# Manta-Network/manta-rs

Hardware: AMD Instinct MI355X
Metric: G1 MSM Mscalar/s at 2^20 (higher is better)
Workload: dtype u32; 1 GPU; 2^20 BLS12-381 G1 variable-base MSM per GPU, uniform scalars resident in HBM; curve=BLS12-381, log_n=20, window_bits=17, msms_in_flight=3

## Files before the change

manta_rs_amd/csrc/ec_dev.h:

```cpp
#pragma once
#include "fp_dev.h"

namespace mg {

#define MG_EC_CALL __device__ __noinline__

template <class F, int B> struct Bv {
    F v;
};
template <int B, class F> MG_DEV Bv<F, B> bv(const F &f) { return Bv<F, B>{f}; }
template <class F, int A, int B> MG_DEV Bv<F, F::BM> operator*(const Bv<F, A> &a, const Bv<F, B> &b) {
    static_assert((long)A * B * F::MULK <= F::LIM, "product of operand bounds exceeds the Montgomery headroom");
    return Bv<F, F::BM>{F::template mulb<A, B>(a.v, b.v)};
}
template <class F, int A> MG_DEV Bv<F, F::BM> b_sqr(const Bv<F, A> &a) {
    static_assert((long)A * A * F::MULK <= F::LIM, "square of operand bound exceeds the Montgomery headroom");
    return Bv<F, F::BM>{F::template sqrb<A>(a.v)};
}
template <class F, int A, int B> MG_DEV Bv<F, A + B> operator+(const Bv<F, A> &a, const Bv<F, B> &b) {
    return Bv<F, A + B>{F::add(a.v, b.v)};
}
template <class F, int A> MG_DEV Bv<F, 2 * A> b_dbl(const Bv<F, A> &a) { return Bv<F, 2 * A>{F::dbl(a.v)}; }
template <class F, int A, int B> MG_DEV Bv<F, A + B> operator-(const Bv<F, A> &a, const Bv<F, B> &b) {
    static_assert(B <= F::MAXM, "no multiple of p large enough for this subtrahend");
    return Bv<F, A + B>{F::template sub<B>(a.v, b.v)};
}
template <class F, int A, int B, int C>
MG_DEV Bv<F, A + B + 2 * C> b_sub2(const Bv<F, A> &a, const Bv<F, B> &b, const Bv<F, C> &c) {
    static_assert(B + 2 * C <= F::MAXM, "no multiple of p large enough for this subtrahend");
    return Bv<F, A + B + 2 * C>{F::template sub2<B + 2 * C>(a.v, b.v, c.v)};
}
template <class F, int A> MG_DEV Bv<F, A> b_neg(const Bv<F, A> &a) {
    static_assert(A <= F::MAXM, "no multiple of p large enough");
    return Bv<F, A>{F::template neg<A>(a.v)};
}
template <class F, int A> MG_DEV bool b_is_zero(const Bv<F, A> &a) {
    static_assert(A - 1 <= F::MAXM, "multiple table too short for this zero test");
    return a.v.template is_zero_mod<A>();
}
template <int T, class F, int A> MG_DEV Bv<F, T> b_fit(const Bv<F, A> &a) {
    if constexpr (A <= T) {
        return Bv<F, T>{a.v};
    } else {
        static_assert(F::BRED <= T, "reduction cannot reach the requested bound");
        return Bv<F, T>{F::template reduce<A>(a.v)};
    }
}

template <class F> struct Affine {
    F x, y;
    MG_DEV bool is_inf() const { return x.is_zero_exact() && y.is_zero_exact(); }
    static MG_DEV Affine load(const u32 *p) { return Affine{F::load_aff(p), F::load_aff(p + F::AFF_N)}; }
    MG_DEV void store(u32 *p) const {
        x.store_aff(p);
        y.store_aff(p + F::AFF_N);
    }
    static constexpr int WORDS = 2 * F::AFF_N;
};

template <class F> struct XYZZ {
    F x, y, zz, zzz;
    static constexpr int WORDS = 4 * F::N;
    static constexpr int BX = F::BX, BY = F::BY, BM = F::BM;
    MG_DEV bool is_inf() const { return zz.is_zero_exact(); }
    static MG_DEV XYZZ inf() { return XYZZ{F::zero(), F::zero(), F::zero(), F::zero()}; }
    static MG_DEV XYZZ from_affine(const Affine<F> &a) {
        if (a.is_inf()) return inf();
        return XYZZ{a.x, a.y, F::one(), F::one()};
    }
    static MG_DEV XYZZ load(const u32 *p) {
        return XYZZ{F::load(p), F::load(p + F::N), F::load(p + 2 * F::N), F::load(p + 3 * F::N)};
    }
    MG_DEV void store(u32 *p) const {
        x.store(p);
        y.store(p + F::N);
        zz.store(p + 2 * F::N);
        zzz.store(p + 3 * F::N);
    }
    MG_DEV void store_std(u32 *p) const {
        typedef typename F::Std S;
        x.to_std().store(p);
        y.to_std().store(p + S::N);
        zz.to_std().store(p + 2 * S::N);
        zzz.to_std().store(p + 3 * S::N);
    }
    static MG_DEV XYZZ shfl(const XYZZ &a, int src) {
        return XYZZ{F::shfl(a.x, src), F::shfl(a.y, src), F::shfl(a.zz, src), F::shfl(a.zzz, src)};
    }
    static MG_DEV XYZZ select(bool c, const XYZZ &a, const XYZZ &b) {
        return XYZZ{F::select(c, a.x, b.x), F::select(c, a.y, b.y), F::select(c, a.zz, b.zz), F::select(c, a.zzz, b.zzz)};
    }

    template <int AX, int AY>
    static MG_DEV void dbl_core(const Bv<F, AX> &px, const Bv<F, AY> &py, F &X3o, F &Y3o, F &Vo, F &Wo) {
        auto U = b_fit<8>(b_dbl(py));
        auto V = b_sqr(U);
        auto W = U * V;
        auto S = px * V;
        auto X2 = b_sqr(px);
        auto M = b_fit<6>(b_dbl(X2) + X2);
        auto X3 = b_fit<BX>(b_sub2(b_sqr(M), bv<0>(F::zero()), S));
        auto Y3 = b_fit<BY>(M * (S - X3) - W * py);
        X3o = X3.v;
        Y3o = Y3.v;
        Vo = V.v;
        Wo = W.v;
    }
    static MG_EC_CALL XYZZ dbl_affine_call(const Affine<F> &p) { return dbl_affine_body(p); }
    static MG_DEV XYZZ dbl_affine(const Affine<F> &p) {
        if constexpr (F::EXT) return dbl_affine_call(p);
        else return dbl_affine_body(p);
    }
    static MG_DEV XYZZ dbl_affine_body(const Affine<F> &p) {
        XYZZ r;
        dbl_core(bv<BM>(p.x), bv<BM>(p.y), r.x, r.y, r.zz, r.zzz);
        return r;
    }
    static MG_EC_CALL XYZZ dbl_call(const XYZZ &p) { return dbl_body(p); }
    static MG_DEV XYZZ dbl(const XYZZ &p) {
        if constexpr (F::EXT) return dbl_call(p);
        else return dbl_body(p);
    }
    static MG_DEV XYZZ dbl_body(const XYZZ &p) {
        if (p.is_inf()) return p;
        XYZZ r;
        F V, W;
        dbl_core(bv<BX>(p.x), bv<BY>(p.y), r.x, r.y, V, W);
        r.zz = (bv<BM>(V) * bv<BM>(p.zz)).v;
        r.zzz = (bv<BM>(W) * bv<BM>(p.zzz)).v;
        return r;
    }
    MG_EC_CALL void madd_call(const Affine<F> &q, bool neg) { madd_body(q, neg); }
    MG_DEV void madd(const Affine<F> &q, bool neg) {
        if constexpr (F::EXT) madd_call(q, neg);
        else madd_body(q, neg);
    }
    MG_DEV void madd_throughput(const Affine<F> &q, bool neg) {
        if constexpr (!F::EXT && F::LAZY) {
#ifdef MG_ACC_TWO_CHAINS
            madd_lazy<false>(q, neg);
#else
            madd_lazy<true>(q, neg);
#endif
            return;
        }
        madd(q, neg);
    }
    template <bool CH = false> MG_DEV void madd_lazy(const Affine<F> &q_in, bool negate) {
        static_assert(!F::EXT && F::LAZY, "reduced-radix base field only");
        static_assert(F::BX == 8 && F::BY == 4 && F::BM == 2 && F::LIM >= 121, "bound analysis above");
        constexpr bool LL = F::LAZY_LIMBS;
        if (q_in.is_inf()) return;
        F qy = q_in.y;
        if (negate) {
            if constexpr (LL) qy = F::template negl<3>(q_in.y);
            else qy = F::template neg<2>(q_in.y);
        }
        if (is_inf()) {
            x = q_in.x;
            y = negate ? F::template neg<2>(q_in.y) : q_in.y;
            zz = F::one();
            zzz = F::one();
            return;
        }
        const F U2 = F::template mul_t<CH>(q_in.x, zz);
        const F S2 = F::template mul_t<CH>(qy, zzz);
        F P, R;
        if constexpr (LL) {
            P = F::template subl<9>(U2, x);
            R = F::template subl<5>(S2, y);
        } else {
            P = F::template sub<8>(U2, x);
            R = F::template sub<4>(S2, y);
        }
        const F PP = F::template sqr_t<CH>(P);
        if (PP.template is_zero_mod<2>()) {
            if ((LL ? F::normalize_u(R) : R).template is_zero_mod<7>()) {
                Affine<F> q{q_in.x, negate ? F::template neg<2>(q_in.y) : q_in.y};
                *this = dbl_affine(q);
            } else {
                *this = inf();
            }
            return;
        }
        const F PPP = F::template mul_t<CH>(P, PP);
        const F Q = F::template mul_t<CH>(x, PP);
        const F X3 = F::template sub2<6>(F::template sqr_t<CH>(R), PPP, Q);
        F T, N;
        if constexpr (LL) {
            T = F::template subl<9>(Q, X3);
            N = F::template negl<3>(PPP);
        } else {
            T = F::template sub<8>(Q, X3);
            N = F::template neg<2>(PPP);
        }
        const F Y3 = F::template mul_add_t<CH>(R, T, y, N);
        zz = F::template mul_t<CH>(zz, PP);
        zzz = F::template mul_t<CH>(zzz, PPP);
        x = X3;
        y = Y3;
    }
    MG_DEV void madd_body(const Affine<F> &q_in, bool negate) {
        if constexpr (!F::EXT && F::LAZY) {
            madd_lazy<false>(q_in, negate);
            return;
        }
        if (q_in.is_inf()) return;
        Affine<F> q = q_in;
        if (negate) q.y = b_neg(bv<BM>(q.y)).v;
        if (is_inf()) {
            x = q.x;
            y = q.y;
            zz = F::one();
            zzz = F::one();
            return;
        }
        const auto X1 = bv<BX>(x);
        const auto Y1 = bv<BY>(y);
        const auto ZZ1 = bv<BM>(zz);
        const auto ZZZ1 = bv<BM>(zzz);
        auto U2 = bv<BM>(q.x) * ZZ1;
        auto S2 = bv<BM>(q.y) * ZZZ1;
        auto P = U2 - X1;
        auto R = S2 - Y1;
        if (b_is_zero(P)) {
            if (b_is_zero(R))
                *this = dbl_affine(q);
            else
                *this = inf();
            return;
        }
        auto PP = b_sqr(P);
        auto PPP = P * PP;
        auto Q = X1 * PP;
        auto X3 = b_fit<BX>(b_sub2(b_sqr(R), PPP, Q));
        auto Y3 = b_fit<BY>(R * (Q - X3) - Y1 * PPP);
        x = X3.v;
        y = Y3.v;
        zz = (ZZ1 * PP).v;
        zzz = (ZZZ1 * PPP).v;
    }
    MG_EC_CALL void add_call(const XYZZ &o) { add_body(o); }
    MG_DEV void add(const XYZZ &o) {
        if constexpr (F::EXT) add_call(o);
        else add_body(o);
    }
    MG_DEV void add_body(const XYZZ &o) {
        if (o.is_inf()) return;
        if (is_inf()) {
            *this = o;
            return;
        }
        auto U1 = bv<BX>(x) * bv<BM>(o.zz);
        auto U2 = bv<BX>(o.x) * bv<BM>(zz);
        auto S1 = bv<BY>(y) * bv<BM>(o.zzz);
        auto S2 = bv<BY>(o.y) * bv<BM>(zzz);
        auto P = U2 - U1;
        auto R = S2 - S1;
        if (b_is_zero(P)) {
            if (b_is_zero(R))
                *this = dbl(*this);
            else
                *this = inf();
            return;
        }
        auto PP = b_sqr(P);
        auto PPP = P * PP;
        auto Q = U1 * PP;
        auto X3 = b_fit<BX>(b_sub2(b_sqr(R), PPP, Q));
        auto Y3 = b_fit<BY>(R * (Q - X3) - S1 * PPP);
        x = X3.v;
        y = Y3.v;
        zz = ((bv<BM>(zz) * bv<BM>(o.zz)) * PP).v;
        zzz = ((bv<BM>(zzz) * bv<BM>(o.zzz)) * PPP).v;
    }
};

template <class F, bool ALLOW_DOUBLE = true> struct CoopAdd {
    static constexpr int SLOT = F::XWORDS;
    static constexpr bool DOUBLE = ALLOW_DOUBLE && 2 * 4 * SLOT * 4 <= 49152;
    static constexpr int LDS_WORDS = (DOUBLE ? 2 : 1) * 4 * SLOT;
    static MG_DEV void swap(u32 *buf, int wave, int lane, const F &mine, F (&all)[4]) {
        mine.store_x(buf + wave * SLOT, lane);
        __syncthreads();
#pragma unroll
        for (int q = 0; q < 4; ++q) all[q] = F::load_x(buf + q * SLOT, lane);
        if (!DOUBLE) __syncthreads();
    }
    static MG_DEV void add(XYZZ<F> &acc, const XYZZ<F> &o, u32 *lds, int wave, int lane) {
        constexpr int BX = F::BX, BY = F::BY, BM = F::BM;
        const bool o_inf = o.is_inf(), a_inf = acc.is_inf();
        F mine, r[4];
        if (wave == 0) mine = (bv<BX>(acc.x) * bv<BM>(o.zz)).v;
        else if (wave == 1) mine = (bv<BX>(o.x) * bv<BM>(acc.zz)).v;
        else if (wave == 2) mine = (bv<BY>(acc.y) * bv<BM>(o.zzz)).v;
        else mine = (bv<BY>(o.y) * bv<BM>(acc.zzz)).v;
        swap(lds, wave, lane, mine, r);
        const auto U1 = bv<BM>(r[0]), U2 = bv<BM>(r[1]), S1 = bv<BM>(r[2]), S2 = bv<BM>(r[3]);
        const auto P = U2 - U1;
        const auto R = S2 - S1;
        const bool p0 = b_is_zero(P), r0 = b_is_zero(R);
        if (wave == 0) mine = b_sqr(P).v;
        else if (wave == 1) mine = b_sqr(R).v;
        else if (wave == 2) mine = (bv<BM>(acc.zz) * bv<BM>(o.zz)).v;
        else mine = (bv<BM>(acc.zzz) * bv<BM>(o.zzz)).v;
        swap(lds + (DOUBLE ? 4 * SLOT : 0), wave, lane, mine, r);
        const auto PP = bv<BM>(r[0]), RR = bv<BM>(r[1]), Z12 = bv<BM>(r[2]), Z123 = bv<BM>(r[3]);
        if (wave == 0) mine = (P * PP).v;
        else if (wave == 1) mine = (U1 * PP).v;
        else if (wave == 2) mine = (Z12 * PP).v;
        else mine = F::zero();
        swap(lds, wave, lane, mine, r);
        const auto PPP = bv<BM>(r[0]), Q = bv<BM>(r[1]);
        const F ZZ3 = r[2];
        const auto X3 = b_fit<BX>(b_sub2(RR, PPP, Q));
        if (wave == 0) mine = (R * (Q - X3)).v;
        else if (wave == 1) mine = (S1 * PPP).v;
        else if (wave == 2) mine = (Z123 * PPP).v;
        else mine = F::zero();
        swap(lds + (DOUBLE ? 4 * SLOT : 0), wave, lane, mine, r);
        const auto Y3 = b_fit<BY>(bv<BM>(r[0]) - bv<BM>(r[1]));
        XYZZ<F> sum{X3.v, Y3.v, ZZ3, r[2]};
        if (o_inf) {
            sum = acc;
        } else if (a_inf) {
            sum = o;
        } else if (p0) {
            if (r0) sum = XYZZ<F>::dbl(acc);
            else sum = XYZZ<F>::inf();
        }
        acc = sum;
    }
};

}
```

manta_rs_amd/csrc/msm_reduce.h:

```cpp
#pragma once
#include "msm_common.h"

namespace mg {

template <class F>
__global__ __launch_bounds__(256) MG_TAIL_ATTR void merge_partials(u32 *__restrict__ pkeys, u32 *__restrict__ ppts, u32 cnt, u32 G,
                                                      u32 invalid, int final_level, u32 *__restrict__ buckets,
                                                      u32 *__restrict__ okeys, u32 *__restrict__ opts, u32 n_waves,
                                                      u32 *__restrict__ std_final) {
    MG_PRIO_FOR(F);
    constexpr size_t XW = XYZZ<F>::WORDS;
    const u32 wave = blockIdx.x * (blockDim.x >> 6) + (threadIdx.x >> 6);
    const int lane = threadIdx.x & 63;
    if (wave >= n_waves) return;
    const size_t b = ((size_t)wave * 64 + lane) * G;
    u32 kh = invalid, kt = invalid;
    bool single = true;
    XYZZ<F> acc = XYZZ<F>::inf();
    if (b < cnt) {
        const size_t end = b + G < cnt ? b + G : cnt;
        u32 cur = pkeys[b];
        if (cur != invalid) {
            kh = cur;
            acc = XYZZ<F>::load(ppts + b * XW);
            for (size_t j = b + 1; j < end; ++j) {
                const u32 k = pkeys[j];
                if (k != cur) {
                    if (single) {
                        acc.store(ppts + b * XW);
                        single = false;
                    } else {
                        acc.store(buckets + (size_t)cur * XW);
                    }
                    cur = k;
                    acc = XYZZ<F>::inf();
                    if (k == invalid) break;
                    acc = XYZZ<F>::load(ppts + j * XW);
                } else {
                    const XYZZ<F> p = XYZZ<F>::load(ppts + j * XW);
                    if (!p.is_inf()) acc.add(p);
                }
            }
            kt = cur;
        }
    }
    for (int d = 1; d < 64; d <<= 1) {
        const u32 nk = __shfl_up(kt, d, 64);
        const bool take = (lane >= d) && (nk == kt) && (kt != invalid);
        if (!__any(take)) break;
        const XYZZ<F> o = XYZZ<F>::shfl(acc, lane - d < 0 ? lane : lane - d);
        if (take) acc.add(o);
    }
    const u32 prev_kt = __shfl_up(kt, 1, 64), next_kh = __shfl_down(kh, 1, 64);
    const u32 key0 = __shfl(kh, 0, 64);
    const bool need_in = !single && lane > 0 && prev_kt == kh;
    const bool any_in = __any(need_in);
    XYZZ<F> prev = XYZZ<F>::inf();
    if (any_in) prev = XYZZ<F>::shfl(acc, lane > 0 ? lane - 1 : 0);
    const bool cont = lane < 63 && next_kh == kt;
    if (kt != invalid && !cont) {
        if (final_level) {
            if (std_final) acc.store_std(std_final + (size_t)kt * XYZZ<typename F::Std>::WORDS);
            else acc.store(buckets + (size_t)kt * XW);
        } else if (kt == key0) {
            okeys[2 * wave] = kt;
            acc.store(opts + (size_t)(2 * wave) * XW);
            if (lane == 63) {
                okeys[2 * wave + 1] = kt;
                XYZZ<F>::inf().store(opts + (size_t)(2 * wave + 1) * XW);
            }
        } else if (lane == 63) {
            okeys[2 * wave + 1] = kt;
            acc.store(opts + (size_t)(2 * wave + 1) * XW);
        } else {
            acc.store(buckets + (size_t)kt * XW);
        }
    }
    if (!final_level && lane == 63 && kt == invalid) {
        okeys[2 * wave + 1] = invalid;
        if (key0 == invalid) okeys[2 * wave] = invalid;
    }
    if (!single) {
        XYZZ<F> h = XYZZ<F>::load(ppts + b * XW);
        if (need_in) h.add(prev);
        if (!final_level && kh == key0) {
            okeys[2 * wave] = kh;
            h.store(opts + (size_t)(2 * wave) * XW);
        } else if (final_level && std_final) {
            h.store_std(std_final + (size_t)kh * XYZZ<typename F::Std>::WORDS);
        } else {
            h.store(buckets + (size_t)kh * XW);
        }
    }
}

template <class F>
__global__ __launch_bounds__(256) MG_TAIL_COOP_ATTR void merge_partials_coop(u32 *__restrict__ pkeys, u32 *__restrict__ ppts, u32 cnt, u32 G,
                                                           u32 invalid, int final_level, u32 *__restrict__ buckets,
                                                           u32 *__restrict__ okeys, u32 *__restrict__ opts,
                                                           u32 *__restrict__ std_final) {
    MG_PRIO_FOR(F);
    __shared__ __attribute__((aligned(16))) u32 lds[CoopAdd<F>::LDS_WORDS];
    constexpr size_t XW = XYZZ<F>::WORDS;
    const u32 wave = blockIdx.x;
    const int lane = threadIdx.x & 63, pw = threadIdx.x >> 6;
    const bool writer = pw == 0;
    const size_t b = ((size_t)wave * 64 + lane) * G;
    u32 kh = invalid, cur = invalid;
    bool single = true, live = false;
    XYZZ<F> acc = XYZZ<F>::inf();
    if (b < cnt) {
        cur = pkeys[b];
        if (cur != invalid) {
            kh = cur;
            acc = XYZZ<F>::load(ppts + b * XW);
            live = true;
        }
    }
    for (u32 off = 1; off < G; ++off) {
        const size_t j = b + off;
        const bool have = live && j < cnt;
        const u32 k = have ? pkeys[j] : invalid;
        XYZZ<F> p = XYZZ<F>::inf();
        if (have && k != invalid) p = XYZZ<F>::load(ppts + j * XW);
        const bool same = have && k == cur;
        if (have && k != cur) {
            if (writer) acc.store(single ? ppts + b * XW : buckets + (size_t)cur * XW);
            single = false;
            cur = k;
            acc = p;
            if (k == invalid) live = false;
        }
        if (__any(same && !p.is_inf())) {
            const XYZZ<F> o = same ? p : XYZZ<F>::inf();
            CoopAdd<F>::add(acc, o, lds, pw, lane);
        }
    }
    const u32 kt = cur;
    __threadfence_block();
    __syncthreads();
    for (int d = 1; d < 64; d <<= 1) {
        const u32 nk = __shfl_up(kt, d, 64);
        const bool take = (lane >= d) && (nk == kt) && (kt != invalid);
        if (!__any(take)) break;
        XYZZ<F> o = XYZZ<F>::shfl(acc, lane - d < 0 ? lane : lane - d);
        if (!take) o = XYZZ<F>::inf();
        CoopAdd<F>::add(acc, o, lds, pw, lane);
    }
    const u32 prev_kt = __shfl_up(kt, 1, 64), next_kh = __shfl_down(kh, 1, 64);
    const u32 key0 = __shfl(kh, 0, 64);
    const bool need_in = !single && lane > 0 && prev_kt == kh;
    const bool any_in = __any(need_in);
    XYZZ<F> prev = XYZZ<F>::inf();
    if (any_in) prev = XYZZ<F>::shfl(acc, lane > 0 ? lane - 1 : 0);
    const bool cont = lane < 63 && next_kh == kt;
    if (writer && kt != invalid && !cont) {
        if (final_level) {
            if (std_final) acc.store_std(std_final + (size_t)kt * XYZZ<typename F::Std>::WORDS);
            else acc.store(buckets + (size_t)kt * XW);
        } else if (kt == key0) {
            okeys[2 * wave] = kt;
            acc.store(opts + (size_t)(2 * wave) * XW);
            if (lane == 63) {
                okeys[2 * wave + 1] = kt;
                XYZZ<F>::inf().store(opts + (size_t)(2 * wave + 1) * XW);
            }
        } else if (lane == 63) {
            okeys[2 * wave + 1] = kt;
            acc.store(opts + (size_t)(2 * wave + 1) * XW);
        } else {
            acc.store(buckets + (size_t)kt * XW);
        }
    }
    if (writer && !final_level && lane == 63 && kt == invalid) {
        okeys[2 * wave + 1] = invalid;
        if (key0 == invalid) okeys[2 * wave] = invalid;
    }
    XYZZ<F> h = XYZZ<F>::inf();
    if (!single) h = XYZZ<F>::load(ppts + b * XW);
    if (any_in) {
        if (!need_in) prev = XYZZ<F>::inf();
        CoopAdd<F>::add(h, prev, lds, pw, lane);
    }
    if (writer && !single) {
        if (!final_level && kh == key0) {
            okeys[2 * wave] = kh;
            h.store(opts + (size_t)(2 * wave) * XW);
        } else if (final_level && std_final) {
            h.store_std(std_final + (size_t)kh * XYZZ<typename F::Std>::WORDS);
        } else {
            h.store(buckets + (size_t)kh * XW);
        }
    }
}

template <class F>
__global__ __launch_bounds__(256) MG_TAIL_ATTR void tile_reduce(const u32 *__restrict__ in, u32 seg_stride ,
                                                   u32 item_off, u32 n_items, u32 tiles_per_seg, u32 n_waves,
                                                   u32 *__restrict__ outA, u32 *__restrict__ outS, int std_out) {
    MG_PRIO_FOR(F);
    const u32 wave = blockIdx.x * (blockDim.x >> 6) + (threadIdx.x >> 6);
    const int lane = threadIdx.x & 63;
    if (wave >= n_waves) return;
    const u32 seg = wave / tiles_per_seg, tile = wave % tiles_per_seg;
    const u32 idx = tile * 64 + lane;
    XYZZ<F> acc = XYZZ<F>::inf();
    if (idx < n_items) acc = XYZZ<F>::load(in + ((size_t)seg * seg_stride + item_off + idx) * XYZZ<F>::WORDS);
    int top = 1;
    {
        const u32 left = n_items - tile * 64;
        const int lim = left < 64 ? (int)left : 64;
        while (top < lim) top <<= 1;
    }
    for (int d = 1; d < top; d <<= 1) {
        const XYZZ<F> o = XYZZ<F>::shfl(acc, lane + d > 63 ? lane : lane + d);
        if (lane + d < 64) acc.add(o);
    }
    constexpr int SW = XYZZ<typename F::Std>::WORDS;
    if (lane == 0) {
        if (std_out)
            acc.store_std(outA + (size_t)wave * SW);
        else
            acc.store(outA + (size_t)wave * XYZZ<F>::WORDS);
    }
    if (outS) {
        for (int d = top >> 1; d >= 1; d >>= 1) {
            const XYZZ<F> o = XYZZ<F>::shfl(acc, lane + d > 63 ? lane : lane + d);
            if (lane < d) acc.add(o);
        }
        if (lane == 0) {
            if (std_out)
                acc.store_std(outS + (size_t)wave * SW);
            else
                acc.store(outS + (size_t)wave * XYZZ<F>::WORDS);
        }
    }
}

template <class F>
__global__ __launch_bounds__(256) MG_SERIAL_ATTR void serial_reduce(const u32 *__restrict__ in, u32 seg_stride , u32 item_off,
                                                     u32 n_items, u32 S, u32 lanes_per_seg, u32 n_lanes,
                                                     u32 *__restrict__ outA, u32 *__restrict__ outS) {
    MG_PRIO_FOR(F);
    constexpr size_t XW = XYZZ<F>::WORDS;
    const u32 g = blockIdx.x * blockDim.x + threadIdx.x;
    if (g >= n_lanes) return;
    const u32 seg = g / lanes_per_seg, l = g % lanes_per_seg;
    const u32 i0 = l * S;
    u32 i1 = i0 + S;
    if (i1 > n_items) i1 = n_items;
    const u32 *base = in + ((size_t)seg * seg_stride + item_off) * XW;
    XYZZ<F> acc = XYZZ<F>::inf(), sum = XYZZ<F>::inf();
    for (u32 i = i1; i-- > i0;) {
        const XYZZ<F> x = XYZZ<F>::load(base + (size_t)i * XW);
        acc.add(x);
        if (outS) sum.add(acc);
    }
    acc.store(outA + (size_t)g * XW);
    if (outS) sum.store(outS + (size_t)g * XW);
}

template <class F>
__global__ __launch_bounds__(256) MG_TAIL_COOP_ATTR void serial_reduce_coop(const u32 *__restrict__ in, u32 seg_stride , u32 item_off,
                                                          u32 n_items, u32 S, u32 lanes_per_seg, u32 n_lanes,
                                                          u32 *__restrict__ outA, u32 *__restrict__ outS) {
    MG_PRIO_FOR(F);
    __shared__ __attribute__((aligned(16))) u32 lds[CoopAdd<F>::LDS_WORDS];
    constexpr size_t XW = XYZZ<F>::WORDS;
    const int lane = threadIdx.x & 63, pw = threadIdx.x >> 6;
    const u32 g = blockIdx.x * 64 + lane;
    const bool live = g < n_lanes;
    const u32 seg = live ? g / lanes_per_seg : 0, l = live ? g % lanes_per_seg : 0;
    const u32 i0 = l * S;
    const u32 *base = in + ((size_t)seg * seg_stride + item_off) * XW;
    XYZZ<F> acc = XYZZ<F>::inf(), sum = XYZZ<F>::inf();
    for (u32 j = S; j-- > 0;) {
        const u32 i = i0 + j;
        XYZZ<F> x = XYZZ<F>::inf();
        if (live && i < n_items) x = XYZZ<F>::load(base + (size_t)i * XW);
        CoopAdd<F>::add(acc, x, lds, pw, lane);
        if (outS) CoopAdd<F>::add(sum, acc, lds, pw, lane);
    }
    if (live && pw == 0) {
        acc.store(outA + (size_t)g * XW);
        if (outS) sum.store(outS + (size_t)g * XW);
    }
}

template <class F>
__global__ __launch_bounds__(256) MG_TAIL_COOP_ATTR void tile_reduce_coop(const u32 *__restrict__ in, u32 seg_stride ,
                                                        u32 item_off, u32 n_items, u32 tiles_per_seg,
                                                        u32 *__restrict__ outA, u32 *__restrict__ outS, int std_out) {
    MG_PRIO_FOR(F);
    __shared__ __attribute__((aligned(16))) u32 lds[CoopAdd<F>::LDS_WORDS];
    const u32 tile_id = blockIdx.x;
    const int lane = threadIdx.x & 63, wave = threadIdx.x >> 6;
    const u32 seg = tile_id / tiles_per_seg, tile = tile_id % tiles_per_seg;
    const u32 idx = tile * 64 + lane;
    XYZZ<F> acc = XYZZ<F>::inf();
    if (idx < n_items) acc = XYZZ<F>::load(in + ((size_t)seg * seg_stride + item_off + idx) * XYZZ<F>::WORDS);
    int top = 1;
    {
        const u32 left = n_items - tile * 64;
        const int lim = left < 64 ? (int)left : 64;
        while (top < lim) top <<= 1;
    }
    for (int d = 1; d < top; d <<= 1) {
        XYZZ<F> o = XYZZ<F>::shfl(acc, lane + d > 63 ? lane : lane + d);
        if (lane + d >= 64) o = XYZZ<F>::inf();
        CoopAdd<F>::add(acc, o, lds, wave, lane);
    }
    constexpr int SW = XYZZ<typename F::Std>::WORDS;
    if (threadIdx.x == 0) {
        if (std_out)
            acc.store_std(outA + (size_t)tile_id * SW);
        else
            acc.store(outA + (size_t)tile_id * XYZZ<F>::WORDS);
    }
    if (outS) {
        for (int d = top >> 1; d >= 1; d >>= 1) {
            XYZZ<F> o = XYZZ<F>::shfl(acc, lane + d > 63 ? lane : lane + d);
            if (lane >= d) o = XYZZ<F>::inf();
            CoopAdd<F>::add(acc, o, lds, wave, lane);
        }
        if (threadIdx.x == 0) {
            if (std_out)
                acc.store_std(outS + (size_t)tile_id * SW);
            else
                acc.store(outS + (size_t)tile_id * XYZZ<F>::WORDS);
        }
    }
}

template <class F>
__global__ __launch_bounds__(128) MG_TAIL_ATTR void reduce_level1(const u32 *__restrict__ A0, const u32 *__restrict__ S0, u32 T0,
                                                     u32 *__restrict__ out_std) {
    MG_PRIO_FOR(F);
    constexpr int XW = XYZZ<F>::WORDS;
    constexpr int SW = XYZZ<typename F::Std>::WORDS;
    const u32 seg = blockIdx.x;
    const int lane = threadIdx.x & 63, wave = threadIdx.x >> 6;
    int top = 1;
    while (top < (int)T0) top <<= 1;
    XYZZ<F> acc = XYZZ<F>::inf();
    if (wave == 0) {
        if (lane >= 1 && lane < (int)T0) acc = XYZZ<F>::load(A0 + ((size_t)seg * T0 + lane) * XW);
        for (int d = 1; d < top; d <<= 1) {
            const XYZZ<F> o = XYZZ<F>::shfl(acc, lane + d > 63 ? lane : lane + d);
            if (lane + d < 64) acc.add(o);
        }
        if (lane == 0) acc = XYZZ<F>::inf();
    } else {
        if (lane < (int)T0) acc = XYZZ<F>::load(S0 + ((size_t)seg * T0 + lane) * XW);
    }
    for (int d = top >> 1; d >= 1; d >>= 1) {
        const XYZZ<F> o = XYZZ<F>::shfl(acc, lane + d > 63 ? lane : lane + d);
        if (lane < d) acc.add(o);
    }
    if (lane == 0) acc.store_std(out_std + ((size_t)seg * 2 + wave) * SW);
}

template <class F>
__global__ __launch_bounds__(256) MG_TAIL_COOP_ATTR void reduce_level1_coop(const u32 *__restrict__ A0, const u32 *__restrict__ S0, u32 T0,
                                                          u32 *__restrict__ out_std) {
    MG_PRIO_FOR(F);
    __shared__ __attribute__((aligned(16))) u32 lds[CoopAdd<F>::LDS_WORDS];
    constexpr int XW = XYZZ<F>::WORDS;
    constexpr int SW = XYZZ<typename F::Std>::WORDS;
    const u32 seg = blockIdx.x >> 1;
    const int part = blockIdx.x & 1;
    const int lane = threadIdx.x & 63, wave = threadIdx.x >> 6;
    int top = 1;
    while (top < (int)T0) top <<= 1;
    XYZZ<F> acc = XYZZ<F>::inf();
    if (part == 0) {
        if (lane >= 1 && lane < (int)T0) acc = XYZZ<F>::load(A0 + ((size_t)seg * T0 + lane) * XW);
        for (int d = 1; d < top; d <<= 1) {
            XYZZ<F> o = XYZZ<F>::shfl(acc, lane + d > 63 ? lane : lane + d);
            if (lane + d >= 64) o = XYZZ<F>::inf();
            CoopAdd<F>::add(acc, o, lds, wave, lane);
        }
        if (lane == 0) acc = XYZZ<F>::inf();
    } else {
        if (lane < (int)T0) acc = XYZZ<F>::load(S0 + ((size_t)seg * T0 + lane) * XW);
    }
    for (int d = top >> 1; d >= 1; d >>= 1) {
        XYZZ<F> o = XYZZ<F>::shfl(acc, lane + d > 63 ? lane : lane + d);
        if (lane >= d) o = XYZZ<F>::inf();
        CoopAdd<F>::add(acc, o, lds, wave, lane);
    }
    if (threadIdx.x == 0) acc.store_std(out_std + ((size_t)seg * 2 + part) * SW);
}

struct FoldDesc {
    const u32 *tail, *extra;
    u32 kind, T1, nP, segs, n_extra, tail_shift;
    u32 extra_shift[8];
};
static_assert(sizeof(FoldDesc::extra_shift) == sizeof(MsmTail::extra_shift), "FoldDesc::extra_shift holds MsmTail::MAX_EXTRA shifts");
template <class F>
__global__ __launch_bounds__(64) void fold_windows(FoldDesc d, u32 *__restrict__ out, size_t out_stride) {
    MG_PRIO_FOR(F);
    typedef typename F::Std S;
    constexpr int SW = XYZZ<S>::WORDS;
    const u32 q = blockIdx.x;
    auto ld = [](const u32 *p) {
        const XYZZ<S> s = XYZZ<S>::load(p);
        if (s.is_inf()) return XYZZ<F>::inf();
        return XYZZ<F>{F::from_std(s.x), F::from_std(s.y), F::from_std(s.zz), F::from_std(s.zzz)};
    };
    auto pow2 = [](XYZZ<F> p, u32 k) {
        for (u32 i = 0; i < k; ++i) p = XYZZ<F>::dbl(p);
        return p;
    };
    XYZZ<F> win = XYZZ<F>::inf();
    if (d.kind == TAIL_WINDOW_SUMS) {
        win = ld(d.tail + (size_t)q * SW);
    } else if (d.kind == TAIL_X_SUMS) {
        win = pow2(ld(d.tail + ((size_t)q * 2 + 0) * SW), 6);
        win.add(ld(d.tail + ((size_t)q * 2 + 1) * SW));
    } else {
        const u32 *A1 = d.tail + (size_t)q * d.T1 * SW;
        const u32 *S1 = d.tail + ((size_t)d.segs * d.T1 + (size_t)q * d.T1) * SW;
        const u32 *P0 = d.tail + ((size_t)d.segs * 2 * d.T1 + (size_t)q * d.nP) * SW;
        XYZZ<F> sumS = XYZZ<F>::inf(), run = XYZZ<F>::inf(), uA = XYZZ<F>::inf();
        for (int u = (int)d.T1 - 1; u >= 0; --u) {
            sumS.add(ld(S1 + (size_t)u * SW));
            if (u >= 1) {
                run.add(ld(A1 + (size_t)u * SW));
                uA.add(run);
            }
        }
        XYZZ<F> X = pow2(uA, 6);
        X.add(sumS);
        win = pow2(X, 6);
        for (u32 u = 0; u < d.nP; ++u) win.add(ld(P0 + (size_t)u * SW));
    }
    if (d.tail_shift) win = pow2(win, d.tail_shift);
    for (u32 e = 0; e < d.n_extra; ++e) win.add(pow2(ld(d.extra + ((size_t)e * d.segs + q) * SW), d.extra_shift[e]));
    if (threadIdx.x == 0) win.store_std(out + (size_t)q * out_stride);
}

}
```

Measured before the change: 403.4 Mscalar/s.

## Keep cooperative tail accumulators in LDS split across waves instead of registers

Adds a CoopAddL helper that holds XYZZ accumulator coordinates in shared memory, with each of four waves owning one coordinate, and rewrites the cooperative merge and reduce tail kernels to use it. Per-thread register copies of full points and the cross-lane shuffles of whole points are replaced by LDS reads at another lane's slot. The goal is lower register pressure and shuffle traffic in the tail kernels. The cost is extra __syncthreads barriers and LDS traffic for every point add.

```diff
diff --git a/manta_rs_amd/csrc/ec_dev.h b/manta_rs_amd/csrc/ec_dev.h
--- a/manta_rs_amd/csrc/ec_dev.h
+++ b/manta_rs_amd/csrc/ec_dev.h
@@ -333,4 +333,114 @@
     }
 };
 
-}
+template <class F> struct CoopAddL {
+    static constexpr int SLOT = F::XWORDS;
+    static constexpr int PT = 4 * SLOT;
+    static constexpr int TMP_SLOTS = 7;
+    static constexpr int TMP = TMP_SLOTS * SLOT;
+    static MG_DEV F ld(const u32 *s, int lane) { return F::load_x(s, lane); }
+    static MG_DEV void st(u32 *s, int lane, const F &v) { v.store_x(s, lane); }
+    static MG_DEV int wave_id() { return __builtin_amdgcn_readfirstlane((int)(threadIdx.x >> 6)); }
+
+    static MG_DEV bool is_inf(const u32 *P, int lane) { return ld(P + 2 * SLOT, lane).is_zero_exact(); }
+    static MG_DEV void set_inf(u32 *P, int wave, int lane) { st(P + wave * SLOT, lane, F::zero()); }
+    static MG_DEV void load(u32 *P, const u32 *g, bool valid, int wave, int lane) {
+        st(P + wave * SLOT, lane, valid ? F::load(g + (size_t)wave * F::N) : F::zero());
+    }
+    static MG_DEV void store(const u32 *P, u32 *g, int wave, int lane) { ld(P + wave * SLOT, lane).store(g + (size_t)wave * F::N); }
+    static MG_DEV void store_std(const u32 *P, u32 *g, int wave, int lane) {
+        typedef typename F::Std S;
+        ld(P + wave * SLOT, lane).to_std().store(g + (size_t)wave * S::N);
+    }
+    static MG_DEV void copy(u32 *D, const u32 *P, int src, int wave, int lane) { st(D + wave * SLOT, lane, ld(P + wave * SLOT, src)); }
+
+    static MG_DEV void add(u32 *A, const u32 *O, int olane, bool take, u32 *T, int wave, int lane) {
+        constexpr int BX = F::BX, BY = F::BY, BM = F::BM;
+        u32 *const ax = A, *const ay = A + SLOT, *const azz = A + 2 * SLOT, *const azzz = A + 3 * SLOT;
+        const u32 *const ox = O, *const oy = O + SLOT, *const ozz = O + 2 * SLOT, *const ozzz = O + 3 * SLOT;
+        u32 *const s0 = T, *const s1 = T + SLOT, *const s2 = T + 2 * SLOT, *const s3 = T + 3 * SLOT, *const s4 = T + 4 * SLOT,
+                   *const s5 = T + 5 * SLOT, *const s6 = T + 6 * SLOT;
+        const bool o_inf = !take || ld(ozz, olane).is_zero_exact();
+        const bool a_inf = ld(azz, lane).is_zero_exact();
+        F keep, sum;
+        if (wave == 0) st(s0, lane, (bv<BX>(ld(ax, lane)) * bv<BM>(ld(ozz, olane))).v);
+        else if (wave == 1) st(s1, lane, (bv<BX>(ld(ox, olane)) * bv<BM>(ld(azz, lane))).v);
+        else if (wave == 2) st(s2, lane, (bv<BY>(ld(ay, lane)) * bv<BM>(ld(ozzz, olane))).v);
+        else st(s3, lane, (bv<BY>(ld(oy, olane)) * bv<BM>(ld(azzz, lane))).v);
+        __syncthreads();
+        bool p0, r0;
+        {
+            const auto P = bv<BM>(ld(s1, lane)) - bv<BM>(ld(s0, lane));
+            p0 = b_is_zero(P);
+            if (wave == 0) keep = P.v;
+        }
+        r0 = b_is_zero(bv<BM>(ld(s3, lane)) - bv<BM>(ld(s2, lane)));
+        if (wave == 0) st(s4, lane, b_sqr(bv<2 * BM>(keep)).v);
+        else if (wave == 1) st(s5, lane, b_sqr(bv<BM>(ld(s3, lane)) - bv<BM>(ld(s2, lane))).v);
+        else if (wave == 2) keep = (bv<BM>(ld(azz, lane)) * bv<BM>(ld(ozz, olane))).v;
+        else keep = (bv<BM>(ld(azzz, lane)) * bv<BM>(ld(ozzz, olane))).v;
+        __syncthreads();
+        if (wave == 0) st(s1, lane, (bv<2 * BM>(keep) * bv<BM>(ld(s4, lane))).v);
+        else if (wave == 1) st(s6, lane, (bv<BM>(ld(s0, lane)) * bv<BM>(ld(s4, lane))).v);
+        else if (wave == 2) sum = (bv<BM>(keep) * bv<BM>(ld(s4, lane))).v;
+        __syncthreads();
+        if (wave == 0) {
+            const auto Q = bv<BM>(ld(s6, lane));
+            const auto X3 = b_fit<BX>(b_sub2(bv<BM>(ld(s5, lane)), bv<BM>(ld(s1, lane)), Q));
+            sum = X3.v;
+            const auto R = bv<BM>(ld(s3, lane)) - bv<BM>(ld(s2, lane));
+            st(s0, lane, (R * (Q - X3)).v);
+        } else if (wave == 1) {
+            sum = (bv<BM>(ld(s2, lane)) * bv<BM>(ld(s1, lane))).v;
+        } else if (wave == 3) {
+            sum = (bv<BM>(keep) * bv<BM>(ld(s1, lane))).v;
+        }
+        __syncthreads();
+        if (wave == 1) sum = b_fit<BY>(bv<BM>(ld(s0, lane)) - bv<BM>(sum)).v;
+        const bool need_dbl = !o_inf && !a_inf && p0 && r0;
+        F dc = F::zero();
+        if (__any(need_dbl))
+            dc = dbl(A, T, wave, lane);
+        if (!o_inf) {
+            F v;
+            if (a_inf) v = ld(O + wave * SLOT, olane);
+            else if (p0) v = r0 ? dc : F::zero();
+            else v = sum;
+            st(A + wave * SLOT, lane, v);
+        }
+        __syncthreads();
+    }
+    static MG_DEV F dbl(const u32 *A, u32 *T, int wave, int lane) {
+        constexpr int BX = F::BX, BY = F::BY, BM = F::BM;
+        const u32 *const ax = A, *const ay = A + SLOT, *const azz = A + 2 * SLOT, *const azzz = A + 3 * SLOT;
+        u32 *const sV = T + SLOT, *const sM = T + 2 * SLOT, *const sW = T + 3 * SLOT, *const sS = T + 4 * SLOT,
+                   *const sMM = T + 5 * SLOT, *const sA = T + 6 * SLOT;
+        F dc = F::zero();
+        if (wave == 0) st(sV, lane, b_sqr(b_fit<8>(b_dbl(bv<BY>(ld(ay, lane))))).v);
+        else if (wave == 1) {
+            const auto X2 = b_sqr(bv<BX>(ld(ax, lane)));
+            st(sM, lane, b_fit<6>(b_dbl(X2) + X2).v);
+        }
+        __syncthreads();
+        if (wave == 0) st(sW, lane, (b_fit<8>(b_dbl(bv<BY>(ld(ay, lane)))) * bv<BM>(ld(sV, lane))).v);
+        else if (wave == 1) st(sS, lane, (bv<BX>(ld(ax, lane)) * bv<BM>(ld(sV, lane))).v);
+        else if (wave == 2) dc = (bv<BM>(ld(sV, lane)) * bv<BM>(ld(azz, lane))).v;
+        else st(sMM, lane, b_sqr(bv<6>(ld(sM, lane))).v);
+        __syncthreads();
+        if (wave == 0) {
+            const auto S = bv<BM>(ld(sS, lane));
+            const auto X3 = b_fit<BX>(b_sub2(bv<BM>(ld(sMM, lane)), bv<0>(F::zero()), S));
+            dc = X3.v;
+            st(sA, lane, (bv<6>(ld(sM, lane)) * (S - X3)).v);
+        } else if (wave == 1) {
+            dc = (bv<BM>(ld(sW, lane)) * bv<BY>(ld(ay, lane))).v;
+        } else if (wave == 3) {
+            dc = (bv<BM>(ld(sW, lane)) * bv<BM>(ld(azzz, lane))).v;
+        }
+        __syncthreads();
+        if (wave == 1) dc = b_fit<BY>(bv<BM>(ld(sA, lane)) - bv<BM>(dc)).v;
+        return dc;
+    }
+};
+
+}
diff --git a/manta_rs_amd/csrc/msm_reduce.h b/manta_rs_amd/csrc/msm_reduce.h
--- a/manta_rs_amd/csrc/msm_reduce.h
+++ b/manta_rs_amd/csrc/msm_reduce.h
@@ -100,41 +100,42 @@
                                                            u32 *__restrict__ okeys, u32 *__restrict__ opts,
                                                            u32 *__restrict__ std_final) {
     MG_PRIO_FOR(F);
-    __shared__ __attribute__((aligned(16))) u32 lds[CoopAdd<F>::LDS_WORDS];
+    typedef CoopAddL<F> C;
+    __shared__ __attribute__((aligned(16))) u32 lds[2 * C::PT + C::TMP];
+    u32 *const A = lds, *const O = lds + C::PT, *const T = lds + 2 * C::PT;
     constexpr size_t XW = XYZZ<F>::WORDS;
+    constexpr int SW = XYZZ<typename F::Std>::WORDS;
     const u32 wave = blockIdx.x;
-    const int lane = threadIdx.x & 63, pw = threadIdx.x >> 6;
+    const int lane = threadIdx.x & 63, pw = C::wave_id();
     const bool writer = pw == 0;
     const size_t b = ((size_t)wave * 64 + lane) * G;
     u32 kh = invalid, cur = invalid;
     bool single = true, live = false;
-    XYZZ<F> acc = XYZZ<F>::inf();
     if (b < cnt) {
         cur = pkeys[b];
         if (cur != invalid) {
             kh = cur;
-            acc = XYZZ<F>::load(ppts + b * XW);
             live = true;
         }
     }
+    C::load(A, ppts + b * XW, live, pw, lane);
     for (u32 off = 1; off < G; ++off) {
         const size_t j = b + off;
         const bool have = live && j < cnt;
         const u32 k = have ? pkeys[j] : invalid;
-        XYZZ<F> p = XYZZ<F>::inf();
-        if (have && k != invalid) p = XYZZ<F>::load(ppts + j * XW);
+        const bool pv = have && k != invalid;
+        const bool p_inf = !pv || F::load(ppts + j * XW + 2 * F::N).is_zero_exact();
+        C::load(O, ppts + j * XW, pv, pw, lane);
         const bool same = have && k == cur;
         if (have && k != cur) {
-            if (writer) acc.store(single ? ppts + b * XW : buckets + (size_t)cur * XW);
+            C::store(A, single ? ppts + b * XW : buckets + (size_t)cur * XW, pw, lane);
             single = false;
             cur = k;
-            acc = p;
+            C::copy(A, O, lane, pw, lane);
             if (k == invalid) live = false;
         }
-        if (__any(same && !p.is_inf())) {
-            const XYZZ<F> o = same ? p : XYZZ<F>::inf();
-            CoopAdd<F>::add(acc, o, lds, pw, lane);
-        }
+        __syncthreads();
+        if (__any(same && !p_inf)) C::add(A, O, lane, same, T, pw, lane);
     }
     const u32 kt = cur;
     __threadfence_block();
@@ -143,53 +144,48 @@
         const u32 nk = __shfl_up(kt, d, 64);
         const bool take = (lane >= d) && (nk == kt) && (kt != invalid);
         if (!__any(take)) break;
-        XYZZ<F> o = XYZZ<F>::shfl(acc, lane - d < 0 ? lane : lane - d);
-        if (!take) o = XYZZ<F>::inf();
-        CoopAdd<F>::add(acc, o, lds, pw, lane);
+        C::add(A, A, lane - d < 0 ? lane : lane - d, take, T, pw, lane);
     }
     const u32 prev_kt = __shfl_up(kt, 1, 64), next_kh = __shfl_down(kh, 1, 64);
     const u32 key0 = __shfl(kh, 0, 64);
     const bool need_in = !single && lane > 0 && prev_kt == kh;
     const bool any_in = __any(need_in);
-    XYZZ<F> prev = XYZZ<F>::inf();
-    if (any_in) prev = XYZZ<F>::shfl(acc, lane > 0 ? lane - 1 : 0);
     const bool cont = lane < 63 && next_kh == kt;
-    if (writer && kt != invalid && !cont) {
+    if (kt != invalid && !cont) {
         if (final_level) {
-            if (std_final) acc.store_std(std_final + (size_t)kt * XYZZ<typename F::Std>::WORDS);
-            else acc.store(buckets + (size_t)kt * XW);
+            if (std_final) C::store_std(A, std_final + (size_t)kt * SW, pw, lane);
+            else C::store(A, buckets + (size_t)kt * XW, pw, lane);
         } else if (kt == key0) {
-            okeys[2 * wave] = kt;
-            acc.store(opts + (size_t)(2 * wave) * XW);
+            if (writer) okeys[2 * wave] = kt;
+            C::store(A, opts + (size_t)(2 * wave) * XW, pw, lane);
             if (lane == 63) {
-                okeys[2 * wave + 1] = kt;
-                XYZZ<F>::inf().store(opts + (size_t)(2 * wave + 1) * XW);
+                if (writer) okeys[2 * wave + 1] = kt;
+                F::zero().store(opts + (size_t)(2 * wave + 1) * XW + (size_t)pw * F::N);
             }
         } else if (lane == 63) {
-            okeys[2 * wave + 1] = kt;
-            acc.store(opts + (size_t)(2 * wave + 1) * XW);
+            if (writer) okeys[2 * wave + 1] = kt;
+            C::store(A, opts + (size_t)(2 * wave + 1) * XW, pw, lane);
         } else {
-            acc.store(buckets + (size_t)kt * XW);
+            C::store(A, buckets + (size_t)kt * XW, pw, lane);
         }
     }
     if (writer && !final_level && lane == 63 && kt == invalid) {
         okeys[2 * wave + 1] = invalid;
         if (key0 == invalid) okeys[2 * wave] = invalid;
     }
-    XYZZ<F> h = XYZZ<F>::inf();
-    if (!single) h = XYZZ<F>::load(ppts + b * XW);
+    C::load(O, ppts + b * XW, !single, pw, lane);
     if (any_in) {
-        if (!need_in) prev = XYZZ<F>::inf();
-        CoopAdd<F>::add(h, prev, lds, pw, lane);
-    }
-    if (writer && !single) {
+        __syncthreads();
+        C::add(O, A, lane > 0 ? lane - 1 : 0, need_in, T, pw, lane);
+    }
+    if (!single) {
         if (!final_level && kh == key0) {
-            okeys[2 * wave] = kh;
-            h.store(opts + (size_t)(2 * wave) * XW);
+            if (writer) okeys[2 * wave] = kh;
+            C::store(O, opts + (size_t)(2 * wave) * XW, pw, lane);
         } else if (final_level && std_final) {
-            h.store_std(std_final + (size_t)kh * XYZZ<typename F::Std>::WORDS);
+            C::store_std(O, std_final + (size_t)kh * SW, pw, lane);
         } else {
-            h.store(buckets + (size_t)kh * XW);
+            C::store(O, buckets + (size_t)kh * XW, pw, lane);
         }
     }
 }
@@ -265,25 +261,28 @@
                                                           u32 n_items, u32 S, u32 lanes_per_seg, u32 n_lanes,
                                                           u32 *__restrict__ outA, u32 *__restrict__ outS) {
     MG_PRIO_FOR(F);
-    __shared__ __attribute__((aligned(16))) u32 lds[CoopAdd<F>::LDS_WORDS];
+    typedef CoopAddL<F> C;
+    __shared__ __attribute__((aligned(16))) u32 lds[3 * C::PT + C::TMP];
+    u32 *const A = lds, *const Sm = lds + C::PT, *const X = lds + 2 * C::PT, *const T = lds + 3 * C::PT;
     constexpr size_t XW = XYZZ<F>::WORDS;
-    const int lane = threadIdx.x & 63, pw = threadIdx.x >> 6;
+    const int lane = threadIdx.x & 63, pw = C::wave_id();
     const u32 g = blockIdx.x * 64 + lane;
     const bool live = g < n_lanes;
     const u32 seg = live ? g / lanes_per_seg : 0, l = live ? g % lanes_per_seg : 0;
     const u32 i0 = l * S;
     const u32 *base = in + ((size_t)seg * seg_stride + item_off) * XW;
-    XYZZ<F> acc = XYZZ<F>::inf(), sum = XYZZ<F>::inf();
+    C::set_inf(A, pw, lane);
+    C::set_inf(Sm, pw, lane);
     for (u32 j = S; j-- > 0;) {
         const u32 i = i0 + j;
-        XYZZ<F> x = XYZZ<F>::inf();
-        if (live && i < n_items) x = XYZZ<F>::load(base + (size_t)i * XW);
-        CoopAdd<F>::add(acc, x, lds, pw, lane);
-        if (outS) CoopAdd<F>::add(sum, acc, lds, pw, lane);
-    }
-    if (live && pw == 0) {
-        acc.store(outA + (size_t)g * XW);
-        if (outS) sum.store(outS + (size_t)g * XW);
+        C::load(X, base + (size_t)i * XW, live && i < n_items, pw, lane);
+        __syncthreads();
+        C::add(A, X, lane, true, T, pw, lane);
+        if (outS) C::add(Sm, A, lane, true, T, pw, lane);
+    }
+    if (live) {
+        C::store(A, outA + (size_t)g * XW, pw, lane);
+        if (outS) C::store(Sm, outS + (size_t)g * XW, pw, lane);
     }
 }
 
@@ -292,42 +291,38 @@
                                                         u32 item_off, u32 n_items, u32 tiles_per_seg,
                                                         u32 *__restrict__ outA, u32 *__restrict__ outS, int std_out) {
     MG_PRIO_FOR(F);
-    __shared__ __attribute__((aligned(16))) u32 lds[CoopAdd<F>::LDS_WORDS];
+    typedef CoopAddL<F> C;
+    __shared__ __attribute__((aligned(16))) u32 lds[C::PT + C::TMP];
+    u32 *const A = lds, *const T = lds + C::PT;
     const u32 tile_id = blockIdx.x;
-    const int lane = threadIdx.x & 63, wave = threadIdx.x >> 6;
+    const int lane = threadIdx.x & 63, wave = C::wave_id();
     const u32 seg = tile_id / tiles_per_seg, tile = tile_id % tiles_per_seg;
     const u32 idx = tile * 64 + lane;
-    XYZZ<F> acc = XYZZ<F>::inf();
-    if (idx < n_items) acc = XYZZ<F>::load(in + ((size_t)seg * seg_stride + item_off + idx) * XYZZ<F>::WORDS);
+    C::load(A, in + ((size_t)seg * seg_stride + item_off + idx) * XYZZ<F>::WORDS, idx < n_items, wave, lane);
+    __syncthreads();
     int top = 1;
     {
         const u32 left = n_items - tile * 64;
         const int lim = left < 64 ? (int)left : 64;
         while (top < lim) top <<= 1;
     }
-    for (int d = 1; d < top; d <<= 1) {
-        XYZZ<F> o = XYZZ<F>::shfl(acc, lane + d > 63 ? lane : lane + d);
-        if (lane + d >= 64) o = XYZZ<F>::inf();
-        CoopAdd<F>::add(acc, o, lds, wave, lane);
-    }
+    for (int d = 1; d < top; d <<= 1)
+        C::add(A, A, lane + d > 63 ? lane : lane + d, lane + d < 64, T, wave, lane);
     constexpr int SW = XYZZ<typename F::Std>::WORDS;
-    if (threadIdx.x == 0) {
+    if (lane == 0) {
         if (std_out)
-            acc.store_std(outA + (size_t)tile_id * SW);
+            C::store_std(A, outA + (size_t)tile_id * SW, wave, lane);
         else
-            acc.store(outA + (size_t)tile_id * XYZZ<F>::WORDS);
+            C::store(A, outA + (size_t)tile_id * XYZZ<F>::WORDS, wave, lane);
     }
     if (outS) {
-        for (int d = top >> 1; d >= 1; d >>= 1) {
-            XYZZ<F> o = XYZZ<F>::shfl(acc, lane + d > 63 ? lane : lane + d);
-            if (lane >= d) o = XYZZ<F>::inf();
-            CoopAdd<F>::add(acc, o, lds, wave, lane);
-        }
-        if (threadIdx.x == 0) {
+        for (int d = top >> 1; d >= 1; d >>= 1)
+            C::add(A, A, lane + d > 63 ? lane : lane + d, lane < d, T, wave, lane);
+        if (lane == 0) {
             if (std_out)
-                acc.store_std(outS + (size_t)tile_id * SW);
+                C::store_std(A, outS + (size_t)tile_id * SW, wave, lane);
             else
-                acc.store(outS + (size_t)tile_id * XYZZ<F>::WORDS);
+                C::store(A, outS + (size_t)tile_id * XYZZ<F>::WORDS, wave, lane);
         }
     }
 }
@@ -364,32 +359,27 @@
 __global__ __launch_bounds__(256) MG_TAIL_COOP_ATTR void reduce_level1_coop(const u32 *__restrict__ A0, const u32 *__restrict__ S0, u32 T0,
                                                           u32 *__restrict__ out_std) {
     MG_PRIO_FOR(F);
-    __shared__ __attribute__((aligned(16))) u32 lds[CoopAdd<F>::LDS_WORDS];
+    typedef CoopAddL<F> C;
+    __shared__ __attribute__((aligned(16))) u32 lds[C::PT + C::TMP];
+    u32 *const A = lds, *const T = lds + C::PT;
     constexpr int XW = XYZZ<F>::WORDS;
     constexpr int SW = XYZZ<typename F::Std>::WORDS;
     const u32 seg = blockIdx.x >> 1;
     const int part = blockIdx.x & 1;
-    const int lane = threadIdx.x & 63, wave = threadIdx.x >> 6;
+    const int lane = threadIdx.x & 63, wave = C::wave_id();
     int top = 1;
     while (top < (int)T0) top <<= 1;
-    XYZZ<F> acc = XYZZ<F>::inf();
     if (part == 0) {
-        if (lane >= 1 && lane < (int)T0) acc = XYZZ<F>::load(A0 + ((size_t)seg * T0 + lane) * XW);
-        for (int d = 1; d < top; d <<= 1) {
-            XYZZ<F> o = XYZZ<F>::shfl(acc, lane + d > 63 ? lane : lane + d);
-            if (lane + d >= 64) o = XYZZ<F>::inf();
-            CoopAdd<F>::add(acc, o, lds, wave, lane);
-        }
-        if (lane == 0) acc = XYZZ<F>::inf();
+        C::load(A, A0 + ((size_t)seg * T0 + lane) * XW, lane >= 1 && lane < (int)T0, wave, lane);
+        __syncthreads();
+        for (int d = 1; d < top; d <<= 1) C::add(A, A, lane + d > 63 ? lane : lane + d, lane + d < 64, T, wave, lane);
+        if (lane == 0) C::set_inf(A, wave, lane);
     } else {
-        if (lane < (int)T0) acc = XYZZ<F>::load(S0 + ((size_t)seg * T0 + lane) * XW);
-    }
-    for (int d = top >> 1; d >= 1; d >>= 1) {
-        XYZZ<F> o = XYZZ<F>::shfl(acc, lane + d > 63 ? lane : lane + d);
-        if (lane >= d) o = XYZZ<F>::inf();
-        CoopAdd<F>::add(acc, o, lds, wave, lane);
-    }
-    if (threadIdx.x == 0) acc.store_std(out_std + ((size_t)seg * 2 + part) * SW);
+        C::load(A, S0 + ((size_t)seg * T0 + lane) * XW, lane < (int)T0, wave, lane);
+    }
+    __syncthreads();
+    for (int d = top >> 1; d >= 1; d >>= 1) C::add(A, A, lane + d > 63 ? lane : lane + d, lane < d, T, wave, lane);
+    if (lane == 0) C::store_std(A, out_std + ((size_t)seg * 2 + part) * SW, wave, lane);
 }
 
 struct FoldDesc {
```

New measurement: 403.3 Mscalar/s (median of 4 runs). No clear change (-0.0%).
